# Qervas/cn_chess_ai

Hardware: AMD Instinct MI355X
Metric: env steps/sec + DQN updates/sec at 8192 parallel games, 1/2/4/8 MI355X (higher is better)
Workload: dtype f32

## Files before the change

cn_chess_ai_amd/csrc/xq_dqn.hip:

```cpp
#include "xq_internal.h"
#include <hip/hip_ext.h>
#include "xq_gemm.hip.h"
#include "xq_screen.hip.h"
#include "xq_gemm_dma.hip.h"
#include "xq_l0grad.hip.h"

#include <algorithm>
#include <cfloat>
#include <cmath>
#include <limits>
#include <mutex>
#include <random>
#include <unordered_map>

struct TdStep; struct ScreenPlan;
namespace xq {
struct TailArgs; struct ClipRecord; struct TdStatsRecord; struct ShadowJob;
struct Screen {
    int mode = XQ_QMAX_FULL;
    int refine_stage = -1;
    DevBuf<uint16_t> wb;
    DevBuf<uint16_t> ab;
    DevBuf<float> p1, p2;
    DevBuf<float> R, na;
// ... 89 lines not shown
    xq::DevBuf<float> qsa, yv, lossv;
    xq::DevBuf<uint32_t> gboards;
    int last_n = 0;
    xq::DevBuf<float> grads_td;  size_t n_grads_td = 0;
    size_t g_w0 = 0, g_wh[XQ_MAX_LAYERS] = {0}, g_wout = 0, g_bh[XQ_MAX_LAYERS] = {0}, g_bout = 0;
    xq::DevBuf<float> grads_full;
    int opt_kind = XQ_OPT_SGD;
    double opt_b1 = 0.9, opt_b2 = 0.999, opt_eps = 1e-8;
    uint64_t opt_t = 0;
    xq::DevBuf<float> adam_m, adam_v;
    double clip_max_norm = 0.0;
    xq::DevBuf<double> clip_partials;
    xq::DevBuf<xq::ClipRecord> clip_rec;
    double target_tau = 0.0;
    bool tgt_rest_synced = false;
    int loss_kind = XQ_LOSS_SQUARED;
    double loss_kappa = 1.0;
    float loss_kappa32 = 1.0f;
    xq::DevBuf<xq::TdStatsRecord> td_stats_rec;
    xq::DevBuf<float> slabs;
    xq::DevBuf<float> slabs_l0;
    xq::DevBuf<uint16_t> l0_planes;
    xq::DevBuf<uint16_t> l0_sel;
    bool l0_split_done = false;
    bool l0_sel_done = false;
    bool l0_mfma = true;
    xq_comm* comm = nullptr;
    bool fused_apply = false;
    struct PendingSlab { const float* src = nullptr; int nslabs = 0; long long stride = 0; };
    PendingSlab pend_w0, pend_hidden[XQ_MAX_LAYERS], pend_wout, pend_bout, pend_bh;
    xq::DevBuf<float> bias_work;
    xq::DevBuf<float> xdense, qfull, tfull;
    xq::DevBuf<uint32_t> hb;
    xq::DevBuf<int32_t> ha;  xq::DevBuf<float> hr;  xq::DevBuf<uint8_t> hd;
    xq::StagedBatch staged;
    int bootstrap = XQ_BOOTSTRAP_ALL;
    xq::DevBuf<float> z96, z96_slabs;
    xq::DevBuf<int> legal_nmoves;
    xq::DevBuf<uint8_t> hside;
    int legal_rows = 0;
    int zero_sum = 0;
    int view = XQ_VIEW_ABSOLUTE;
    xq::Profiler prof;
    xq::TailArgs* tail = nullptr;
    bool tail_open = false;
    bool td_tail = true;
// ... 496 lines not shown
    }
    if (kept) { K.valid = true; K.boards = boards_dev; K.n = n; }
    *q90_dev = q;
    *q_stride = 96;
    return XQ_OK;
}

static int check_reference_topology(const xq_dqn* d) {
    for (int l = d->nl - 2; l >= 0; --l) {
        const int inputSize = d->L[l + 1], outputSize = d->L[l];
        if (d->L[l + 2] < inputSize || outputSize < d->L[l + 1] ||
            d->wo[l + 1] + (size_t)(inputSize - 1) * outputSize + (size_t)(d->L[l + 1] - 1) >= d->nw)
            return fail(XQ_ERR_UNDEFINED_UPSTREAM,
                        "bug-compatible backprop reads out of bounds upstream for this topology (layer %d)", l);
    }
    return XQ_OK;
}

static bool l0_mfma_shape(const xq_dqn* d, int n) { return d->l0_mfma && (d->L[1] % 64) == 0 && n >= 256; }
static int l0_chunk_of(int n) { return n >= 16384 ? 2048 : 1024; }
static int ensure_l0_mfma(xq_dqn* d, int n) {
    const int H = d->L[1], chunk = l0_chunk_of(n), kpad = (n + chunk - 1) / chunk * chunk;
    XQ_TRY(reserve_zeroed(d->l0_planes, l0m_plane_elems(H, kpad), d->cur));
    return reserve_zeroed(d->l0_sel, l0sel_elems(kpad), d->cur);
}

static bool grad_bf16_ok(const xq_dqn* d, int M, int N, int K);
static int hidden_deltas(xq_dqn* d, int n, const float* dnext, int ld_next, int k_nz, int mode, int l_start = -1, int l_stop = 0) {
    const float* up = dnext;
    int ld_up = ld_next, nz = k_nz;
    if (l_start < 0) l_start = d->nl - 2;
    for (int l = l_start; l >= l_stop; --l) {
        GemmArgs g; memset(&g, 0, sizeof g);
        g.M = n; g.N = d->L[l + 1];
        const int kfull = (mode == XQ_BACKPROP_REFERENCE) ? d->L[l + 1] : d->L[l + 2];
        g.K = std::min(kfull, nz);
        if (d->bf16_bwd() && up == d->deltas[l + 1] && (n % kBgBM) == 0 && (g.N % kBgBN) == 0 && (g.K % kBgBK) == 0) {
            Bf16GemmArgs b; memset(&b, 0, sizeof b);
            b.M = n; b.N = g.N; b.K = g.K; b.k_chunk = b.K;
            b.A = d->deltas_bf[l + 1]; b.lda = ld_up;
            b.B = d->wl_bf(XQ_NET_ONLINE, l + 1); b.ldb = (mode == XQ_BACKPROP_REFERENCE) ? d->L[l] : d->L[l + 1];
            b.C = d->deltas[l]; b.ldc = d->L[l + 1];
            b.Cb = d->deltas_bf[l]; b.ldcb = d->L[l + 1];
            b.Hb = d->acts_bf[l]; b.ldh = d->L[l + 1];
            XQ_TRY((launch_bf16_gemm<L_KCONTIG, L_MCONTIG, BG_DELTA>(d, b, 1, "gemm_hidden_delta")));
            up = d->deltas[l]; ld_up = d->L[l + 1]; nz = d->L[l + 1];
// ... 127 lines not shown
    s.lds = (size_t)s.nsets * 14 * s.HS * sizeof(float) + (size_t)chunk * sizeof(uint16_t);
    return s;
}

static int l0_gradient(xq_dqn* d, int n, float* dst, xq_dqn::PendingSlab* defer) {
    const int H = d->L[1];
    const int chunk = l0_chunk_of(n);
    const int nchunks = (n + chunk - 1) / chunk;
    const long long len = (long long)kStateSize * H;
    float* out = dst;
    if (nchunks > 1) {
        XQ_TRY(d->slabs_l0.reserve((size_t)nchunks * (size_t)len));
        out = d->slabs_l0;
    }
    if (l0_mfma_shape(d, n)) {
        const int kpad = nchunks * chunk;
        XQ_TRY(ensure_l0_mfma(d, n));
        const size_t need_sel = l0sel_elems(kpad);
        const long long plane_stride = (long long)H * kpad;
        {
            LaunchNow now(d);
            if (!d->l0_sel_done) {
                ProfScope ps(d, "l0_sel_words", 0.0, (double)n * 48 + 2.0 * need_sel);
                hipLaunchKernelGGL(l0_sel_kernel, dim3(kpad / 64), dim3(256), 0, d->cur, d->gboards, n, kpad, d->l0_sel);
            }
            if (!d->l0_split_done) {
                ProfScope ps(d, "l0_delta_split", 8.0 * n * H, (double)n * H * 4 + 6.0 * H * kpad);
                hipLaunchKernelGGL(delta_split_kernel, dim3(kpad / 64, H / 64), dim3(256), 0, d->cur, d->deltas[0], n, H, d->l0_planes, plane_stride, kpad);
            }
            d->l0_sel_done = d->l0_split_done = false;
        }
        XQ_HIP(hipGetLastError());
        const size_t shmem = l0m_lds_bytes();
        const double fl = 2.0 * 80 * 16 * (double)H * kpad * 3, by = 6.0 * H * kpad + 2.0 * need_sel + 4.0 * nchunks * len;
        if (d->tail_open) {
            TailArgs& T = *d->tail;
            T.l0_n = n; T.l0_H = H; T.l0_chunk = chunk; T.l0_nch = nchunks; T.l0_partial = out;
            T.l0_sel = d->l0_sel; T.l0_planes = d->l0_planes; T.l0_plane_stride = plane_stride; T.l0_kpad = kpad; T.l0_ncb = H / kL0mCols;
            T.n_l0 = 4 * (H / kL0mCols) * nchunks;
            d->tail_flops += fl; d->tail_bytes += by;
            d->tail_lds = std::max(d->tail_lds, shmem);
        } else {
            ProfScope ps(d, "l0_grad_segsum", fl, by);
            XQ_TRY(ensure_max_dynamic_lds(l0_grad_mfma_kernel<0>, 64 * 1024));
            hipLaunchKernelGGL(l0_grad_mfma_kernel<0>, dim3(H / kL0mCols, 4, nchunks), dim3(256), shmem, d->cur, d->l0_sel, d->l0_planes, plane_stride,
                               kpad, H, chunk, out);
            XQ_HIP(hipGetLastError());
        }
    } else {
        ProfScope ps(d, "l0_grad_segsum", 2.0 * n * 32 * H, (double)n * (32.0 * H * 4 + 48) + 4.0 * nchunks * len);
        const L0SegShape shape = l0_seg_shape(H, chunk);
        const int HS = shape.HS, nsets = shape.nsets;
        const size_t shmem = shape.lds;
        if (d->tail_open) {
            TailArgs& T = *d->tail;
            T.l0_boards = d->gboards; T.l0_delta = d->deltas[0]; T.l0_n = n; T.l0_H = H; T.l0_HS = HS; T.l0_chunk = chunk; T.l0_nsets = nsets;
            T.l0_nch = nchunks; T.l0_partial = out; T.n_l0 = kSquares * nchunks * (H / HS);
            d->tail_flops += 2.0 * n * 32 * H; d->tail_bytes += (double)n * (32.0 * H * 4 + 48) + 4.0 * nchunks * len;
            d->tail_lds = std::max(d->tail_lds, shmem);
        } else {
        if (shmem > 48 * 1024) XQ_TRY(ensure_max_dynamic_lds(l0_grad_kernel, 64 * 1024));
        hipLaunchKernelGGL(l0_grad_kernel, dim3(kSquares, nchunks, H / HS), dim3(256), shmem, d->cur, d->gboards, d->deltas[0], n, H, HS,
// ... 561 lines not shown
static int side_gradients(xq_dqn* d, const GradPlan& P, int n, float* const* outs, float* G) {
    const int nl = d->nl;
    XQ_TRY(out_gradient(d, P, n, outs[nl - 2], G));
    bool waited = false;
    for (int l = nl - 2; l >= 1; --l) {
        if (l < nl - 2 && !waited) { XQ_HIP(hipStreamWaitEvent(d->cur, d->ev_delta, 0)); waited = true; }
        XQ_TRY(hidden_weight_gradient(d, P, l, n, outs, G));
    }
    if (!waited) XQ_HIP(hipStreamWaitEvent(d->cur, d->ev_delta, 0));
    return hidden_bias_gradients(d, P, n, G);
}

struct TailGrid {
    xq_dqn* d;
    explicit TailGrid(xq_dqn* d_) : d(d_) {
        if (!d->tail) d->tail = new TailArgs();
        memset(d->tail, 0, sizeof(TailArgs));
        d->tail_open = true; d->tail_lds = 0; d->tail_flops = d->tail_bytes = 0;
    }
    ~TailGrid() { d->tail_open = false; }
    int launch(bool last, const char* name) {
        d->tail_open = false;
        const TailArgs& T = *d->tail;
        const long long total = (long long)T.n_l0 + T.n_grad + T.n_delta + T.n_out + T.n_colsum + T.n_sel;
        if (total <= 0) return XQ_OK;
        ProfScope ps(d, name, d->tail_flops, d->tail_bytes, true);
        const auto kern = last ? (T.l0_planes != nullptr ? td_tail_kernel<TAIL_L0 | TAIL_GRAD | TAIL_OUT | TAIL_COLSUM, true>
                                                         : td_tail_kernel<TAIL_L0 | TAIL_GRAD | TAIL_OUT | TAIL_COLSUM>)
                               : (T.n_sel ? td_tail_kernel<TAIL_GRAD | TAIL_DELTA | TAIL_OUT | TAIL_SEL> : td_tail_kernel<TAIL_GRAD | TAIL_DELTA | TAIL_OUT>);
        if (d->tail_lds > 48 * 1024) XQ_TRY(ensure_max_dynamic_lds(kern, 64 * 1024));
        hipExtLaunchKernelGGL(kern, dim3((unsigned)total), dim3(256), d->tail_lds, d->cur, ps.start(), ps.stop(), 0, T);
        XQ_HIP(hipGetLastError());
        return XQ_OK;
    }
};
static bool tail_eligible(xq_dqn* d, int n) {
    if (!d->td_tail || d->bf16()) return false;
    for (int l = 0; l + 2 < d->nl; ++l)
        if (!d->small_tiles && (long long)((n + 127) / 128) * ((d->L[l + 1] + 127) / 128) >= 512) return false;
    return true;
}
static int reduce_pending(xq_dqn* d) {
    SegTable t; memset(&t, 0, sizeof t);
    float* G = d->grads_td;
    int k = 0;
    for_td_segments(d, [&](float*, uint16_t*, size_t goff, long long len, xq_dqn::PendingSlab& p) {
        if (p.nslabs > 0) { t.dst[k] = G + goff; t.src[k] = p.src; t.len[k] = len; t.nslabs[k] = p.nslabs; t.stride[k] = p.stride; ++k; }
        p = xq_dqn::PendingSlab();
    });
    if (k == 0) return XQ_OK;
    t.nseg = k; t.reduce_only = 1;
    return sgd_apply(d, t, 0.0);
}
static int tail_launches(xq_dqn* d, int n, float* const* outs, float* G, int mode) {
    const int nl = d->nl;
    GradPlan P;
    XQ_TRY(plan_gradients(d, n, true, &P));
    const bool defer_grad = nl == 3;
    int waiting = -1;
    for (int l = nl - 3; l >= 0; --l) {
        TailGrid grid(d);
        XQ_TRY(hidden_deltas(d, n, d->deltas[l + 1], d->L[l + 2], d->L[l + 2], mode, l, l));
        if (defer_grad) { if (waiting >= 0) XQ_TRY(hidden_weight_gradient(d, P, waiting, n, outs, G)); waiting = l + 1; }
        else XQ_TRY(hidden_weight_gradient(d, P, l + 1, n, outs, G));
        if (l == nl - 3) XQ_TRY(out_gradient(d, P, n, outs[nl - 2], G));
        if (l == 0 && l0_mfma_shape(d, n)) {
            XQ_TRY(ensure_l0_mfma(d, n));
            TailArgs& T = *d->tail;
            const int chunk0 = l0_chunk_of(n), kpad = (n + chunk0 - 1) / chunk0 * chunk0;
            T.sel_boards = d->gboards; T.sel_n = n; T.sel_kpad = kpad; T.sel_out = d->l0_sel; T.n_sel = kpad / 64;
            d->tail_bytes += (double)n * 48 + 2.0 * l0sel_elems(kpad);
            d->tail_lds = std::max(d->tail_lds, (size_t)64 * 13 * sizeof(uint32_t));
            d->l0_sel_done = true;
        }
        XQ_TRY(grid.launch(false, "td_tail_deltas"));
    }
    TailGrid grid(d);
    XQ_TRY(l0_gradient(d, n, G + d->g_w0, &d->pend_w0));
    if (waiting >= 0) XQ_TRY(hidden_weight_gradient(d, P, waiting, n, outs, G));
    if (nl < 3) XQ_TRY(out_gradient(d, P, n, outs[nl - 2], G));
    XQ_TRY(hidden_bias_gradients(d, P, n, G));
    return grid.launch(true, "td_tail_l0");
}
static int tail_gradients(xq_dqn* d, int n, float* const* outs, float* G, int mode) {
    int rc = tail_launches(d, n, outs, G, mode);
    if (d->late_gate) {
        if (hipEventRecord(d->ev_qmax, d->stream) != hipSuccess && rc == XQ_OK) rc = fail(XQ_ERR_RUNTIME, "hipEventRecord failed");
    }
    if (rc == XQ_OK && !d->fused()) {
        rc = reduce_pending(d);
        if (rc == XQ_OK && d->comm) {
            ProfScope ps(d, "rccl_allreduce_grads", 0, 4.0 * d->n_grads_td);
            rc = comm_allreduce_on(d->comm, G, d->n_grads_td, d->stream);
// ... 1096 lines not shown
```

cn_chess_ai_amd/csrc/xq_l0grad.hip.h:

```cpp
#pragma once

#include "xq_gemm.hip.h"

namespace xq {

constexpr int kL0mRS = 5;
constexpr int kL0mRC = 2;
constexpr int kL0mRowsB = 4 * kL0mRS * 16;
constexpr int kL0mSqB = 24;
constexpr int kL0mCols = 16 * kL0mRC;
constexpr int kL0mStageK = 64;
constexpr int kL0mAPieces = 2 * 3 * kL0mRC;
constexpr int kL0mSPieces = 2 * 3;
constexpr int kL0mStageB = (kL0mAPieces + kL0mSPieces) * 1024;
constexpr int kL0mStages = 3;
constexpr int kL0mSelSquares = 96;

__host__ __device__ constexpr size_t l0m_plane_elems(int H, int kpad) { return (size_t)3 * H * kpad + 8 * 32 + 64; }
__host__ __device__ constexpr size_t l0m_lds_bytes() { return (size_t)kL0mStages * kL0mStageB; }
__host__ __device__ constexpr size_t l0sel_elems(int kpad) { return (size_t)kL0mSelSquares * kpad * 2 + 1024; }

__device__ __forceinline__ void l0_sel_block(const uint32_t* __restrict__ gboards, int n, int kpad, uint16_t* __restrict__ sel, int blk,
                                             uint32_t* __restrict__ bw ) {
    const int tid = (int)threadIdx.x, b0 = blk * 64;
    for (int i = tid; i < 64 * kBoardWords; i += 256) {
        const int s = i / kBoardWords, w = i - s * kBoardWords;
        bw[s * 13 + w] = b0 + s < n ? gboards[(long long)(b0 + s) * kBoardWords + w] : 0u;
    }
    __syncthreads();
    const int octs = kpad >> 3;
    for (int p = tid; p < kL0mSelSquares * 16; p += 256) {
        const int sq = p >> 4, oct = (p >> 1) & 7, enc = p & 1;
        const int wd = sq >> 3, sh = 4 * (sq & 7);
        uint32_t o[4];
#pragma unroll
        for (int i2 = 0; i2 < 4; ++i2) {
            uint32_t v = 0;
#pragma unroll
            for (int e = 0; e < 2; ++e) {
                const uint32_t c = (bw[(oct * 8 + 2 * i2 + e) * 13 + wd] >> sh) & 15u;
                const uint32_t idx = enc ? (c >= 8u ? c - 7u : 0u) : (c <= 7u ? c : 0u);
                v |= idx << (8 + 16 * e);
            }
            o[i2] = v;
        }
        *reinterpret_cast<uint4*>(sel + (((long long)sq * octs + (b0 >> 3) + oct) * 2 + enc) * 8) = make_uint4(o[0], o[1], o[2], o[3]);
    }
}
__global__ __launch_bounds__(256) void l0_sel_kernel(const uint32_t* __restrict__ gboards, int n, int kpad, uint16_t* __restrict__ sel) {
    __shared__ uint32_t bw[64 * 13];
    l0_sel_block(gboards, n, kpad, sel, (int)blockIdx.x, bw);
}

__device__ __forceinline__ void delta_split_block(const float* __restrict__ d0, int n, int H, uint16_t* __restrict__ planes,
                                                   long long plane_stride, int kpad, int tile_k, int tile_c, float* __restrict__ tile ) {
    const int tid = (int)threadIdx.x;
    const int k0 = tile_k * 64, c0 = tile_c * 64;
    {
        const int r = tid >> 4, c4 = (tid & 15) * 4;
#pragma unroll
        for (int i = 0; i < 4; ++i) {
            const int k = k0 + r + 16 * i;
            float4 x = make_float4(0.f, 0.f, 0.f, 0.f);
            if (k < n) x = *reinterpret_cast<const float4*>(d0 + (long long)k * H + c0 + c4);
            float* p = tile + (r + 16 * i) * 65 + c4;
            p[0] = x.x; p[1] = x.y; p[2] = x.z; p[3] = x.w;
        }
    }
    __syncthreads();
    const int col = tid >> 2, kq = (tid & 3) * 16;
    uint32_t w[3][8];
#pragma unroll
    for (int j = 0; j < 16; j += 2) {
        uint32_t pk[3] = {0u, 0u, 0u};
// ... 2 lines not shown
            const float v = tile[(kq + j + e) * 65 + col];
            const uint16_t hi = bf16_bits(0.5f * v);
            const float r1 = 0.5f * v - bf16_to_float(hi);
            const uint16_t mid = bf16_bits(r1);
            const float r2 = r1 - bf16_to_float(mid);
            const uint16_t lo = bf16_bits(r2);
            pk[0] |= (uint32_t)hi << (16 * e); pk[1] |= (uint32_t)mid << (16 * e); pk[2] |= (uint32_t)lo << (16 * e);
        }
        w[0][j >> 1] = pk[0]; w[1][j >> 1] = pk[1]; w[2][j >> 1] = pk[2];
    }
#pragma unroll
    for (int t = 0; t < 3; ++t) {
        uint4* o = reinterpret_cast<uint4*>(planes + t * plane_stride + (long long)(c0 + col) * kpad + k0 + kq);
        o[0] = make_uint4(w[t][0], w[t][1], w[t][2], w[t][3]);
        o[1] = make_uint4(w[t][4], w[t][5], w[t][6], w[t][7]);
    }
}
__global__ __launch_bounds__(256) void delta_split_kernel(const float* __restrict__ d0, int n, int H, uint16_t* __restrict__ planes,
                                                           long long plane_stride, int kpad) {
    __shared__ float tile[64 * 65];
    delta_split_block(d0, n, H, planes, plane_stride, kpad, (int)blockIdx.x, (int)blockIdx.y, tile);
}

template <int DBG = 0>
__device__ __forceinline__ void l0_grad_mfma_block(const uint16_t* __restrict__ sel, const uint16_t* __restrict__ planes,
                                                    long long plane_stride, int kpad, int H, int chunk, float* __restrict__ partial,
                                                    int sqg, int cb, int ch, unsigned char* __restrict__ smem) {
    const int tid = (int)threadIdx.x, lane = tid & 63, wid = __builtin_amdgcn_readfirstlane(tid >> 6);
    const int m = lane & 15, g = lane >> 4;
    const int c0 = ch * chunk, octs = kpad >> 3;
    const unsigned lds0 = (unsigned)(size_t)((__attribute__((address_space(3))) unsigned char*)smem);
    unsigned voff[5];
    int piece[5];
    {
        const int col = lane >> 2, kq = (lane & 3) ^ ((col >> 1) & 3);
#pragma unroll
        for (int i = 0; i < 3; ++i) {
            const int p = wid + 4 * i, kk = p / 6, r = p - 6 * kk, t = r >> 1, c16 = r & 1;
            piece[i] = p;
            voff[i] = (unsigned)((t * plane_stride + (long long)(cb * kL0mCols + c16 * 16 + col) * kpad + c0 + kk * 32 + kq * 8) * 2);
        }
#pragma unroll
        for (int i = 3; i < 5; ++i) {
            const int sp = i == 3 ? wid : 4 + (wid & 1), kk = sp / 3, q = sp - 3 * kk;
            piece[i] = kL0mAPieces + sp;
            const int sq = (sqg * kL0mRowsB) / 14 + q * 8 + (lane >> 3), gg = (lane >> 1) & 3, enc = lane & 1;
            voff[i] = (unsigned)((((long long)sq * octs + (c0 >> 3) + kk * 4 + gg) * 2 + enc) * 16);
        }
    }
    const unsigned char* pA = reinterpret_cast<const unsigned char*>(planes);
    const unsigned char* pS = reinterpret_cast<const unsigned char*>(sel);
    auto issue1 = [&](int st, unsigned buf_off, int i) {
        unsigned keep;
        const unsigned char* base = i < 3 ? pA + (long long)st * (kL0mStageK * 2) : pS + (long long)st * (kL0mStageK / 8 * 32);
        const unsigned l = lds0 + buf_off + (unsigned)piece[i] * 1024u;
        asm volatile("s_mov_b32 %0, m0\n\ts_mov_b32 m0, %3\n\ts_nop 0\n\tglobal_load_lds_dwordx4 %1, %2\n\ts_mov_b32 m0, %0"
                     : "=&s"(keep) : "v"(voff[i]), "s"(base), "s"(l) : "memory");
    };
    auto issue = [&](int st, unsigned buf_off) {
#pragma unroll
        for (int i = 0; i < 5; ++i) issue1(st, buf_off, i);
    };
    issue(0, 0u);
    f32x4 acc[kL0mRC][kL0mRS];
#pragma unroll
    for (int c = 0; c < kL0mRC; ++c)
#pragma unroll
        for (int j = 0; j < kL0mRS; ++j) acc[c][j] = f32x4{0.f, 0.f, 0.f, 0.f};
    uint32_t tlo[kL0mRS], thi[kL0mRS];
    unsigned soff[kL0mRS];
    const unsigned aoff = (unsigned)(m * 64 + ((g ^ ((m >> 1) & 3)) << 4));
    const int sq0 = (sqg * kL0mRowsB) / 14;
#pragma unroll
    for (int j = 0; j < kL0mRS; ++j) {
        const int r = sqg * kL0mRowsB + (wid * kL0mRS + j) * 16 + m;
        const int sq = r / 14, pl = r - sq * 14;
        const int enc = pl >= 7 ? 1 : 0;
        const int idx = r >= kStateSize ? 8 : (enc ? pl - 6 : pl + 1);
        tlo[j] = idx < 4 ? 0x40u << (8 * idx) : 0u;
        thi[j] = (idx >= 4 && idx < 8) ? 0x40u << (8 * (idx - 4)) : 0u;
        const int sl = min(sq - sq0, kL0mSqB - 1);
        soff[j] = (unsigned)((kL0mAPieces + (sl >> 3)) * 1024 + (sl & 7) * 128 + g * 32 + enc * 16);
    }
    struct Frags { bf16x8 a[kL0mRC][3]; uint4 sw[kL0mRS]; };
    constexpr int kReads = 6 + kL0mRS;
    auto read_frag = [&](Frags& f, unsigned boff, int kk, int i) {
        const unsigned char* sp = smem + boff;
        constexpr int kind[kReads] = {0, 1, 1, 0, 1, 1, 0, 1, 1, 0, 0};
        constexpr int arg[kReads] = {0, 0, 1, 1, 2, 3, 2, 4, 5, 3, 4};
        if (kind[i] == 0) f.sw[arg[i]] = *reinterpret_cast<const uint4*>(sp + kk * 3 * 1024 + soff[arg[i]]);
        else f.a[arg[i] & 1][arg[i] >> 1] = *reinterpret_cast<const bf16x8*>(sp + (kk * 6 + arg[i]) * 1024 + aoff);
    };
    auto read_frags = [&](Frags& f, unsigned boff, int kk) {
#pragma unroll
        for (int i = 0; i < kReads; ++i) read_frag(f, boff, kk, i);
    };
    auto onehot2 = [&](int j, uint32_t x, uint32_t y, uint32_t& ox, uint32_t& oy) {
        if (DBG == 3 || DBG == 6) { ox = x; oy = y; }
        else { ox = __builtin_amdgcn_perm(thi[j], tlo[j], x); oy = __builtin_amdgcn_perm(thi[j], tlo[j], y); }
    };
    auto kstep = [&](const Frags& f, const Frags& nxt, uint4& o, auto&& side) {
#pragma unroll
        for (int j = 0; j < kL0mRS; ++j) {
            const bf16x8 b = __builtin_bit_cast(bf16x8, o);
            const uint4 nx = j + 1 < kL0mRS ? f.sw[j + 1] : nxt.sw[0];
            const int jn = j + 1 < kL0mRS ? j + 1 : 0;
            uint4 on;
            if (DBG == 2) {
                asm volatile("" : "+v"(acc[0][j]), "+v"(acc[1][j]) : "v"(f.a[0][0]), "v"(f.a[1][0]), "v"(f.a[0][1]), "v"(f.a[1][1]), "v"(f.a[0][2]), "v"(f.a[1][2]), "v"(b));
                onehot2(jn, nx.x, nx.y, on.x, on.y); onehot2(jn, nx.z, nx.w, on.z, on.w);
                side(3 * j); side(3 * j + 1); side(3 * j + 2);
            } else {
                asm volatile("v_mfma_f32_16x16x32_bf16 %0, %2, %4, %0\n\tv_mfma_f32_16x16x32_bf16 %1, %3, %4, %1"
// ... 8 lines not shown
                __builtin_amdgcn_sched_barrier(0);
                asm volatile("v_mfma_f32_16x16x32_bf16 %0, %2, %4, %0\n\tv_mfma_f32_16x16x32_bf16 %1, %3, %4, %1"
                             : "+v"(acc[0][j]), "+v"(acc[1][j]) : "v"(f.a[0][2]), "v"(f.a[1][2]), "v"(b));
                side(3 * j + 2);
                __builtin_amdgcn_sched_barrier(0);
            }
            o = on;
        }
    };
    const int nst = DBG == 1 ? 0 : chunk / kL0mStageK;
    issue(1, (unsigned)kL0mStageB);
    asm volatile("s_waitcnt vmcnt(5)" ::: "memory");
    __builtin_amdgcn_s_barrier();
    asm volatile("" ::: "memory");
    Frags f0, f1;
    read_frags(f0, 0u, 0);
    if (DBG == 6) read_frags(f1, 0u, 1);
    uint4 o;
    onehot2(0, f0.sw[0].x, f0.sw[0].y, o.x, o.y);
    onehot2(0, f0.sw[0].z, f0.sw[0].w, o.z, o.w);
    asm volatile("s_nop 1" : "+v"(o.x), "+v"(o.y), "+v"(o.z), "+v"(o.w));
    unsigned b_cur = 0u, b_nxt = (unsigned)kL0mStageB, b_far = 2u * kL0mStageB;
    for (int st = 0; st < nst; ++st) {
        kstep(f0, f1, o, [&](int p) {
            if (DBG == 6) return;
            if (p < kReads) read_frag(f1, b_cur, 1, p);
            else if (p < kReads + 4 && DBG != 4) issue1(st + 2, b_far, p - kReads);
        });
        if (DBG != 4 && DBG != 6) asm volatile("s_waitcnt vmcnt(4)" ::: "memory");
        asm volatile("s_waitcnt lgkmcnt(0)" ::: "memory");
        __builtin_amdgcn_s_barrier();
        asm volatile("" ::: "memory");
        kstep(f1, f0, o, [&](int p) {
            if (DBG == 6) return;
            if (p < kReads) read_frag(f0, b_nxt, 0, p);
            else if (p == kReads && DBG != 4) issue1(st + 2, b_far, 4);
        });
        const unsigned t = b_cur; b_cur = b_nxt; b_nxt = b_far; b_far = t;
    }
    asm volatile("s_waitcnt vmcnt(0)\n\ts_nop 7\n\ts_nop 7" ::: "memory");
    {
        float* out = partial + ((long long)ch * kStateSize) * H;
#pragma unroll
        for (int j = 0; j < kL0mRS; ++j) {
            const int r = sqg * kL0mRowsB + (wid * kL0mRS + j) * 16 + m;
            if (r >= kStateSize) continue;
#pragma unroll
            for (int c = 0; c < kL0mRC; ++c) {
                const f32x4 v = acc[c][j];
                *reinterpret_cast<float4*>(out + (long long)r * H + cb * kL0mCols + 16 * c + 4 * g) = make_float4(v[0], v[1], v[2], v[3]);
            }
        }
    }
}

template <int DBG = 0>
__global__ __launch_bounds__(256) void l0_grad_mfma_kernel(const uint16_t* __restrict__ sel, const uint16_t* __restrict__ planes,
                                                            long long plane_stride, int kpad, int H, int chunk, float* __restrict__ partial) {
    extern __shared__ __attribute__((aligned(1024))) unsigned char l0m_smem[];
    l0_grad_mfma_block<DBG>(sel, planes, plane_stride, kpad, H, chunk, partial, (int)blockIdx.y, (int)blockIdx.x, (int)blockIdx.z, l0m_smem);
}

}
```

cn_chess_ai_amd/csrc/xq_tail.hip.h:

```cpp
#pragma once

namespace xq {

__device__ __forceinline__ void out_grad_block(const int32_t* __restrict__ act, const float* __restrict__ dsc,
                                               const float* __restrict__ a_last, int n, int H, int chunk,
                                               float* __restrict__ partial, int g , int chunk_id, float* __restrict__ smem) {
    float* acc = smem;
    uint16_t* list = reinterpret_cast<uint16_t*>(smem + 16 * H);
    __shared__ int total;
    __shared__ float bsum[4][4];
    const int c0 = chunk_id * chunk, c1 = min(n, c0 + chunk);
    const int tid = (int)threadIdx.x, lane = tid & 63, wid = tid >> 6;
    constexpr int kMaxIters = 8;
    __shared__ int wc[kMaxIters][4];
    int clsv[kMaxIters];
#pragma unroll
    for (int it = 0; it < kMaxIters; ++it) {
        const int b = c0 + it * 256 + tid;
        const int a = act[min(b, c1 - 1)];
        clsv[it] = (b < c1 && a >= 4 * g && a < 4 * g + 4) ? a - 4 * g : -1;
    }
    for (int i = tid; i < 16 * H; i += 256) acc[i] = 0.f;
#pragma unroll
    for (int it = 0; it < kMaxIters; ++it) {
// ... 123 lines not shown
    colsum_partial_block(J, (int)blockIdx.x, (int)blockIdx.y, (int)blockIdx.z);
}
__global__ __launch_bounds__(256) void colsum_final_kernel(ColsumJobs J) {
    __shared__ float red[4][64];
    const int job = (int)blockIdx.y;
    const int C = J.C[job];
    const int tx = (int)(threadIdx.x & 63), ty = (int)(threadIdx.x >> 6);
    const int c = (int)blockIdx.x * 64 + tx;
    if ((int)blockIdx.x * 64 >= C) return;
    float s0 = 0.f;
    if (c < C) {
        const float* p = J.work + J.poff[job] + c;
        const int R4 = J.R & ~3;
        for (int z = ty; z < R4; z += 4) s0 += p[(long long)z * J.wld];
        if (ty == 0) for (int z = R4; z < J.R; ++z) s0 += p[(long long)z * J.wld];
    }
    red[ty][tx] = s0;
    __syncthreads();
    if (ty == 0 && c < C) J.dst[job][c] = (red[0][tx] + red[1][tx]) + (red[2][tx] + red[3][tx]);
}

enum { TAIL_DELTA = 1, TAIL_GRAD = 2, TAIL_OUT = 4, TAIL_COLSUM = 8, TAIL_L0 = 16, TAIL_SEL = 32 };
struct TailArgs {
    int n_l0, n_grad, n_delta, n_out, n_colsum, n_sel;
    GemmArgs grad;  int grad_gx, grad_gy;
    GemmArgs delta; int delta_gx;
    const int32_t* og_act; const float* og_dsc; const float* og_alast; int og_n, og_H, og_chunk; float* og_partial;
    const uint32_t* l0_boards; const float* l0_delta; int l0_n, l0_H, l0_HS, l0_chunk, l0_nsets, l0_nch; float* l0_partial;
    const uint16_t* l0_planes; long long l0_plane_stride; int l0_kpad, l0_ncb;
    const uint16_t* l0_sel;
    const uint32_t* sel_boards; int sel_n, sel_kpad; uint16_t* sel_out;
    ColsumJobs cj; int cj_gx, cj_gy;
};
template <unsigned KINDS, bool L0MFMA = false>
__global__ __launch_bounds__(256) void td_tail_kernel(const TailArgs a) {
    extern __shared__ __attribute__((aligned(16))) float tail_smem[];
    int b = (int)blockIdx.x;
    if (KINDS & TAIL_L0) {
        if (b < a.n_l0) {
            if (L0MFMA) {
                int rest = b / a.l0_ncb, cb = b % a.l0_ncb, sqg = rest & 3, ch = rest >> 2;
                if ((a.l0_nch & 7) == 0) { ch = b % a.l0_nch; rest = b / a.l0_nch; cb = rest % a.l0_ncb; sqg = rest / a.l0_ncb; }
                l0_grad_mfma_block<0>(a.l0_sel, a.l0_planes, a.l0_plane_stride, a.l0_kpad, a.l0_H, a.l0_chunk, a.l0_partial, sqg, cb, ch,
                                       reinterpret_cast<unsigned char*>(tail_smem));
                return;
            }
            const int per = kSquares * a.l0_nch;
            l0_grad_block(a.l0_boards, a.l0_delta, a.l0_n, a.l0_H, a.l0_HS, a.l0_chunk, a.l0_nsets, a.l0_partial, b % per, a.l0_nch, b / per, tail_smem);
            return;
        }
        b -= a.n_l0;
    }
    if (KINDS & TAIL_GRAD) {
        if (b < a.n_grad) {
            const int per = a.grad_gx * a.grad_gy, nz = a.n_grad / per, z = b % nz, r = b / nz;
            gemm_f32_block<L_MCONTIG, L_MCONTIG, EPI_STORE, 1, 1>(a.grad, r % a.grad_gx, r / a.grad_gx, z, tail_smem, tail_smem + g_tile_floats(64));
            return;
        }
        b -= a.n_grad;
    }
    if (KINDS & TAIL_DELTA) {
        if (b < a.n_delta) {
            gemm_f32_block<L_KCONTIG, L_MCONTIG, EPI_DELTA, 1, 1>(a.delta, b % a.delta_gx, b / a.delta_gx, 0, tail_smem, tail_smem + g_tile_floats(64));
            return;
        }
        b -= a.n_delta;
    }
    if (KINDS & TAIL_OUT) {
        if (b < a.n_out) {
            out_grad_block(a.og_act, a.og_dsc, a.og_alast, a.og_n, a.og_H, a.og_chunk, a.og_partial, b % 24, b / 24, tail_smem);
            return;
        }
        b -= a.n_out;
    }
    if (KINDS & TAIL_COLSUM) {
        if (b < a.n_colsum) {
            const int per = a.cj_gx * a.cj_gy, r = b % per;
            colsum_partial_block(a.cj, r % a.cj_gx, r / a.cj_gx, b / per);
            return;
        }
        b -= a.n_colsum;
    }
    if (KINDS & TAIL_SEL) {
        if (b < a.n_sel) l0_sel_block(a.sel_boards, a.sel_n, a.sel_kpad, a.sel_out, b, reinterpret_cast<uint32_t*>(tail_smem));
    }
}

}
```

Measured before the change: 49.43 million.

## Restrict layer-0 MFMA gradient to reachable piece-square rows, handle cold rows sparsely

Builds a host table of piece/square input rows that are reachable from the start position under movement rules. The fused-tail layer-0 gradient MFMA kernel then runs over 3 packed groups of hot rows instead of 4 groups covering all 1260 rows. Samples that touch unreachable rows are listed per block, and a small sparse kernel accumulates those rows, or zeroes them when none occur. This cuts MFMA work and adds bookkeeping in the selection kernel plus a new cold-path kernel and pipeline-slot changes.

Measured after the change: 49.98 million, median of 6. 1.01x the previous value.

```diff
diff --git a/cn_chess_ai_amd/csrc/xq_dqn.hip b/cn_chess_ai_amd/csrc/xq_dqn.hip
--- a/cn_chess_ai_amd/csrc/xq_dqn.hip
+++ b/cn_chess_ai_amd/csrc/xq_dqn.hip
@@ -135,6 +135,10 @@
     xq::DevBuf<float> slabs_l0;
     xq::DevBuf<uint16_t> l0_planes;
     xq::DevBuf<uint16_t> l0_sel;
+    xq::DevBuf<uint16_t> l0_hot;
+    xq::DevBuf<uint16_t> l0_cold_list;
+    xq::DevBuf<int> l0_cold_cnt;
+    const xq::L0HotTable* hot() const { return reinterpret_cast<const xq::L0HotTable*>(l0_hot.p); }
     bool l0_split_done = false;
     bool l0_sel_done = false;
     bool l0_mfma = true;
@@ -677,6 +681,14 @@
 static int ensure_l0_mfma(xq_dqn* d, int n) {
     const int H = d->L[1], chunk = l0_chunk_of(n), kpad = (n + chunk - 1) / chunk * chunk;
     XQ_TRY(reserve_zeroed(d->l0_planes, l0m_plane_elems(H, kpad), d->cur));
+    if (!d->l0_hot.p) {
+        const L0HotTable& t = l0_hot_table();
+        if (!t.ok) return fail(XQ_ERR_RUNTIME, "hot-row table: the reachable rows do not fit %d groups of %d", kL0HotGroups, kL0HotGroupRows);
+        XQ_TRY(d->l0_hot.reserve(sizeof(L0HotTable) / sizeof(uint16_t)));
+        XQ_HIP(hipMemcpyAsync(d->l0_hot.p, &t, sizeof t, hipMemcpyHostToDevice, d->cur));
+    }
+    XQ_TRY(d->l0_cold_list.reserve(l0cold_elems(kpad)));
+    XQ_TRY(d->l0_cold_cnt.reserve((size_t)kpad / 64));
     return reserve_zeroed(d->l0_sel, l0sel_elems(kpad), d->cur);
 }
 
@@ -850,7 +862,8 @@
             LaunchNow now(d);
             if (!d->l0_sel_done) {
                 ProfScope ps(d, "l0_sel_words", 0.0, (double)n * 48 + 2.0 * need_sel);
-                hipLaunchKernelGGL(l0_sel_kernel, dim3(kpad / 64), dim3(256), 0, d->cur, d->gboards, n, kpad, d->l0_sel);
+                hipLaunchKernelGGL(l0_sel_kernel, dim3(kpad / 64), dim3(256), 0, d->cur, d->gboards, n, kpad, d->l0_sel, d->hot(), d->l0_cold_list.p,
+                                   d->l0_cold_cnt.p);
             }
             if (!d->l0_split_done) {
                 ProfScope ps(d, "l0_delta_split", 8.0 * n * H, (double)n * H * 4 + 6.0 * H * kpad);
@@ -859,13 +872,17 @@
             d->l0_sel_done = d->l0_split_done = false;
         }
         XQ_HIP(hipGetLastError());
-        const size_t shmem = l0m_lds_bytes();
-        const double fl = 2.0 * 80 * 16 * (double)H * kpad * 3, by = 6.0 * H * kpad + 2.0 * need_sel + 4.0 * nchunks * len;
+        const bool hot = d->tail_open;
+        const size_t shmem = hot ? l0m_lds_bytes<true>() : l0m_lds_bytes<false>();
+        const double fl = 2.0 * (hot ? kL0HotGroups * kL0HotGroupRows : 80 * 16) * (double)H * kpad * 3,
+                     by = 6.0 * H * kpad + 2.0 * need_sel + 4.0 * nchunks * len;
         if (d->tail_open) {
             TailArgs& T = *d->tail;
             T.l0_n = n; T.l0_H = H; T.l0_chunk = chunk; T.l0_nch = nchunks; T.l0_partial = out;
             T.l0_sel = d->l0_sel; T.l0_planes = d->l0_planes; T.l0_plane_stride = plane_stride; T.l0_kpad = kpad; T.l0_ncb = H / kL0mCols;
-            T.n_l0 = 4 * (H / kL0mCols) * nchunks;
+            T.n_l0 = kL0HotGroups * (H / kL0mCols) * nchunks;
+            T.l0_hot = d->hot(); T.l0_cold_list = d->l0_cold_list; T.l0_cold_cnt = d->l0_cold_cnt; T.l0_delta = d->deltas[0];
+            T.n_l0cold = kL0ColdParts * nchunks;
             d->tail_flops += fl; d->tail_bytes += by;
             d->tail_lds = std::max(d->tail_lds, shmem);
         } else {
@@ -1473,7 +1490,7 @@
     int launch(bool last, const char* name) {
         d->tail_open = false;
         const TailArgs& T = *d->tail;
-        const long long total = (long long)T.n_l0 + T.n_grad + T.n_delta + T.n_out + T.n_colsum + T.n_sel;
+        const long long total = (long long)T.n_l0 + T.n_grad + T.n_delta + T.n_out + T.n_colsum + T.n_sel + T.n_l0cold;
         if (total <= 0) return XQ_OK;
         ProfScope ps(d, name, d->tail_flops, d->tail_bytes, true);
         const auto kern = last ? (T.l0_planes != nullptr ? td_tail_kernel<TAIL_L0 | TAIL_GRAD | TAIL_OUT | TAIL_COLSUM, true>
@@ -1520,6 +1537,7 @@
             TailArgs& T = *d->tail;
             const int chunk0 = l0_chunk_of(n), kpad = (n + chunk0 - 1) / chunk0 * chunk0;
             T.sel_boards = d->gboards; T.sel_n = n; T.sel_kpad = kpad; T.sel_out = d->l0_sel; T.n_sel = kpad / 64;
+            T.l0_hot = d->hot(); T.sel_cold_list = d->l0_cold_list; T.sel_cold_cnt = d->l0_cold_cnt;
             d->tail_bytes += (double)n * 48 + 2.0 * l0sel_elems(kpad);
             d->tail_lds = std::max(d->tail_lds, (size_t)64 * 13 * sizeof(uint32_t));
             d->l0_sel_done = true;
diff --git a/cn_chess_ai_amd/csrc/xq_l0grad.hip.h b/cn_chess_ai_amd/csrc/xq_l0grad.hip.h
--- a/cn_chess_ai_amd/csrc/xq_l0grad.hip.h
+++ b/cn_chess_ai_amd/csrc/xq_l0grad.hip.h
@@ -1,37 +1,52 @@
 #pragma once
 
 #include "xq_gemm.hip.h"
+#include "xq_l0hot.h"
 
 namespace xq {
 
-constexpr int kL0mRS = 5;
+template <bool HOT> struct L0mShape {
+    static constexpr int kRS = HOT ? 4 : 5;
+    static constexpr int kRowsB = 4 * kRS * 16;
+    static constexpr int kGroups = HOT ? kL0HotGroups : 4;
+    static constexpr int kSqB = HOT ? kL0HotSqB : 24;
+    static constexpr int kSQ = kSqB / 8;
+    static constexpr int kSPieces = 2 * kSQ;
+    static constexpr int kStageB = (2 * 3 * 2 + kSPieces) * 1024;
+};
+static_assert(L0mShape<true>::kRowsB == kL0HotGroupRows, "the table packs what a block computes");
 constexpr int kL0mRC = 2;
-constexpr int kL0mRowsB = 4 * kL0mRS * 16;
-constexpr int kL0mSqB = 24;
 constexpr int kL0mCols = 16 * kL0mRC;
 constexpr int kL0mStageK = 64;
 constexpr int kL0mAPieces = 2 * 3 * kL0mRC;
-constexpr int kL0mSPieces = 2 * 3;
-constexpr int kL0mStageB = (kL0mAPieces + kL0mSPieces) * 1024;
 constexpr int kL0mStages = 3;
 constexpr int kL0mSelSquares = 96;
 
 __host__ __device__ constexpr size_t l0m_plane_elems(int H, int kpad) { return (size_t)3 * H * kpad + 8 * 32 + 64; }
-__host__ __device__ constexpr size_t l0m_lds_bytes() { return (size_t)kL0mStages * kL0mStageB; }
+template <bool HOT = false> __host__ __device__ constexpr size_t l0m_lds_bytes() { return (size_t)kL0mStages * L0mShape<HOT>::kStageB; }
 __host__ __device__ constexpr size_t l0sel_elems(int kpad) { return (size_t)kL0mSelSquares * kpad * 2 + 1024; }
 
+constexpr int kL0ColdCap = 64 * kSquares;
+constexpr int kL0ColdParts = 8;
+__host__ __device__ constexpr size_t l0cold_elems(int kpad) { return (size_t)(kpad / 64) * kL0ColdCap; }
+
 __device__ __forceinline__ void l0_sel_block(const uint32_t* __restrict__ gboards, int n, int kpad, uint16_t* __restrict__ sel, int blk,
-                                             uint32_t* __restrict__ bw ) {
+                                             uint32_t* __restrict__ bw , const L0HotTable* __restrict__ hot,
+                                             uint16_t* __restrict__ cold_list, int* __restrict__ cold_cnt) {
     const int tid = (int)threadIdx.x, b0 = blk * 64;
+    __shared__ uint16_t hm[kL0mSelSquares];
+    if (tid < kL0mSelSquares) hm[tid] = hot ? hot->hot_mask[tid] : (uint16_t)0x3FFF;
     for (int i = tid; i < 64 * kBoardWords; i += 256) {
         const int s = i / kBoardWords, w = i - s * kBoardWords;
         bw[s * 13 + w] = b0 + s < n ? gboards[(long long)(b0 + s) * kBoardWords + w] : 0u;
     }
     __syncthreads();
     const int octs = kpad >> 3;
+    uint32_t any_cold = 0;
     for (int p = tid; p < kL0mSelSquares * 16; p += 256) {
         const int sq = p >> 4, oct = (p >> 1) & 7, enc = p & 1;
         const int wd = sq >> 3, sh = 4 * (sq & 7);
+        const uint32_t coldp = ~((uint32_t)hm[sq] >> (7 * enc)) << 1;
         uint32_t o[4];
 #pragma unroll
         for (int i2 = 0; i2 < 4; ++i2) {
@@ -41,15 +56,89 @@
                 const uint32_t c = (bw[(oct * 8 + 2 * i2 + e) * 13 + wd] >> sh) & 15u;
                 const uint32_t idx = enc ? (c >= 8u ? c - 7u : 0u) : (c <= 7u ? c : 0u);
                 v |= idx << (8 + 16 * e);
+                any_cold |= idx ? (coldp >> idx) & 1u : 0u;
             }
             o[i2] = v;
         }
         *reinterpret_cast<uint4*>(sel + (((long long)sq * octs + (b0 >> 3) + oct) * 2 + enc) * 8) = make_uint4(o[0], o[1], o[2], o[3]);
     }
-}
-__global__ __launch_bounds__(256) void l0_sel_kernel(const uint32_t* __restrict__ gboards, int n, int kpad, uint16_t* __restrict__ sel) {
+    if (!hot) return;
+    if (!__syncthreads_or((int)any_cold)) {
+        if (tid == 0) cold_cnt[blk] = 0;
+        return;
+    }
+    __shared__ int cc[256];
+    const int s = tid >> 2, sqa = (tid & 3) * 23, sqb = min(kSquares, sqa + 23);
+    auto cold_at = [&](int sq) -> int {
+        const uint32_t c = (bw[s * 13 + (sq >> 3)] >> (4 * (sq & 7))) & 15u;
+        if (c == 0u || c == 15u) return -1;
+        const uint32_t cold_planes = ~(uint32_t)hm[sq] & 0x3FFFu;
+        if (!((cold_planes >> (c - 1u)) & 1u)) return -1;
+        return (int)hot->cold_base[sq] + __popc(cold_planes & ((1u << (c - 1u)) - 1u));
+    };
+    int mine = 0;
+    for (int sq = sqa; sq < sqb; ++sq) mine += cold_at(sq) >= 0;
+    cc[tid] = mine;
+    __syncthreads();
+    int off = 0;
+    for (int i = 0; i < tid; ++i) off += cc[i];
+    uint16_t* lst = cold_list + (long long)blk * kL0ColdCap;
+    for (int sq = sqa; sq < sqb; ++sq) {
+        const int ci = cold_at(sq);
+        if (ci >= 0) lst[off++] = (uint16_t)((s << 10) | ci);
+    }
+    if (tid == 255) cold_cnt[blk] = off;
+}
+__global__ __launch_bounds__(256) void l0_sel_kernel(const uint32_t* __restrict__ gboards, int n, int kpad, uint16_t* __restrict__ sel,
+                                                      const L0HotTable* __restrict__ hot, uint16_t* __restrict__ cold_list,
+                                                      int* __restrict__ cold_cnt) {
     __shared__ uint32_t bw[64 * 13];
-    l0_sel_block(gboards, n, kpad, sel, (int)blockIdx.x, bw);
+    l0_sel_block(gboards, n, kpad, sel, (int)blockIdx.x, bw, hot, cold_list, cold_cnt);
+}
+
+__device__ __forceinline__ void l0_cold_block(const L0HotTable* __restrict__ hot, const uint16_t* __restrict__ cold_list,
+                                              const int* __restrict__ cold_cnt, const float* __restrict__ d0, int H, int chunk,
+                                              float* __restrict__ partial, int ch, int part, int nparts) {
+    const int tid = (int)threadIdx.x, lane = tid & 63, wid = tid >> 6;
+    const int nb = chunk / 64, b0 = ch * nb;
+    int total = 0;
+    for (int i = 0; i < nb; ++i) total += cold_cnt[b0 + i];
+    const int ncold = hot->n_cold, per = (ncold + nparts - 1) / nparts, lo = part * per, hi = min(ncold, lo + per);
+    float* out = partial + (long long)ch * kStateSize * H;
+    if (total == 0) {
+        const int q4 = H >> 2;
+        for (int i = tid; i < (hi - lo) * q4; i += 256) {
+            const int r = hot->cold_row[lo + i / q4];
+            *reinterpret_cast<float4*>(out + (long long)r * H + (i % q4) * 4) = make_float4(0.f, 0.f, 0.f, 0.f);
+        }
+        return;
+    }
+    for (int ci = lo + wid; ci < hi; ci += 4) {
+        const int r = hot->cold_row[ci];
+        for (int cbase = 0; cbase < H; cbase += 256) {
+            const int col = cbase + lane * 4;
+            const bool active = col < H;
+            float4 acc = make_float4(0.f, 0.f, 0.f, 0.f);
+            for (int i = 0; i < nb; ++i) {
+                const int cnt = cold_cnt[b0 + i];
+                const uint16_t* lst = cold_list + (long long)(b0 + i) * kL0ColdCap;
+                for (int e0 = 0; e0 < cnt; e0 += 64) {
+                    const int e = e0 + lane < cnt ? (int)lst[e0 + lane] : 0xFFFF;
+                    unsigned long long mask = __ballot((e & 1023) == ci);
+                    while (mask) {
+                        const int l = __builtin_ctzll(mask);
+                        mask &= mask - 1ull;
+                        const int smp = (b0 + i) * 64 + (__shfl(e, l) >> 10);
+                        if (active) {
+                            const float4 x = *reinterpret_cast<const float4*>(d0 + (long long)smp * H + col);
+                            acc.x += x.x; acc.y += x.y; acc.z += x.z; acc.w += x.w;
+                        }
+                    }
+                }
+            }
+            if (active) *reinterpret_cast<float4*>(out + (long long)r * H + col) = acc;
+        }
+    }
 }
 
 __device__ __forceinline__ void delta_split_block(const float* __restrict__ d0, int n, int H, uint16_t* __restrict__ planes,
@@ -98,10 +187,13 @@
     delta_split_block(d0, n, H, planes, plane_stride, kpad, (int)blockIdx.x, (int)blockIdx.y, tile);
 }
 
-template <int DBG = 0>
+template <int DBG = 0, bool HOT = false>
 __device__ __forceinline__ void l0_grad_mfma_block(const uint16_t* __restrict__ sel, const uint16_t* __restrict__ planes,
                                                     long long plane_stride, int kpad, int H, int chunk, float* __restrict__ partial,
-                                                    int sqg, int cb, int ch, unsigned char* __restrict__ smem) {
+                                                    int sqg, int cb, int ch, unsigned char* __restrict__ smem,
+                                                    const L0HotTable* __restrict__ hot = nullptr) {
+    using Sh = L0mShape<HOT>;
+    constexpr int kL0mRS = Sh::kRS, kL0mRowsB = Sh::kRowsB, kL0mSqB = Sh::kSqB, kL0mSQ = Sh::kSQ, kL0mStageB = Sh::kStageB;
     const int tid = (int)threadIdx.x, lane = tid & 63, wid = __builtin_amdgcn_readfirstlane(tid >> 6);
     const int m = lane & 15, g = lane >> 4;
     const int c0 = ch * chunk, octs = kpad >> 3;
@@ -118,9 +210,10 @@
         }
 #pragma unroll
         for (int i = 3; i < 5; ++i) {
-            const int sp = i == 3 ? wid : 4 + (wid & 1), kk = sp / 3, q = sp - 3 * kk;
+            const int sp = i == 3 ? wid : 4 + (HOT ? wid : (wid & 1)), kk = sp / kL0mSQ, q = sp - kL0mSQ * kk;
             piece[i] = kL0mAPieces + sp;
-            const int sq = (sqg * kL0mRowsB) / 14 + q * 8 + (lane >> 3), gg = (lane >> 1) & 3, enc = lane & 1;
+            const int sqb = HOT ? (int)hot->sq0[sqg] : (sqg * kL0mRowsB) / 14;
+            const int sq = min(sqb + q * 8 + (lane >> 3), kL0mSelSquares - 1), gg = (lane >> 1) & 3, enc = lane & 1;
             voff[i] = (unsigned)((((long long)sq * octs + (c0 >> 3) + kk * 4 + gg) * 2 + enc) * 16);
         }
     }
@@ -146,11 +239,12 @@
     uint32_t tlo[kL0mRS], thi[kL0mRS];
     unsigned soff[kL0mRS];
     const unsigned aoff = (unsigned)(m * 64 + ((g ^ ((m >> 1) & 3)) << 4));
-    const int sq0 = (sqg * kL0mRowsB) / 14;
+    const int sq0 = HOT ? (int)hot->sq0[sqg] : (sqg * kL0mRowsB) / 14;
 #pragma unroll
     for (int j = 0; j < kL0mRS; ++j) {
-        const int r = sqg * kL0mRowsB + (wid * kL0mRS + j) * 16 + m;
-        const int sq = r / 14, pl = r - sq * 14;
+        const int pr = sqg * kL0mRowsB + (wid * kL0mRS + j) * 16 + m;
+        const int r = HOT ? (int)hot->row[pr] : pr;
+        const int sq = r >= kStateSize ? sq0 : r / 14, pl = r >= kStateSize ? 0 : r - sq * 14;
         const int enc = pl >= 7 ? 1 : 0;
         const int idx = r >= kStateSize ? 8 : (enc ? pl - 6 : pl + 1);
         tlo[j] = idx < 4 ? 0x40u << (8 * idx) : 0u;
@@ -160,11 +254,12 @@
     }
     struct Frags { bf16x8 a[kL0mRC][3]; uint4 sw[kL0mRS]; };
     constexpr int kReads = 6 + kL0mRS;
+    static_assert(kL0mRS == 4 || kL0mRS == 5, "the read order below lists tiles 0..4");
     auto read_frag = [&](Frags& f, unsigned boff, int kk, int i) {
         const unsigned char* sp = smem + boff;
-        constexpr int kind[kReads] = {0, 1, 1, 0, 1, 1, 0, 1, 1, 0, 0};
-        constexpr int arg[kReads] = {0, 0, 1, 1, 2, 3, 2, 4, 5, 3, 4};
-        if (kind[i] == 0) f.sw[arg[i]] = *reinterpret_cast<const uint4*>(sp + kk * 3 * 1024 + soff[arg[i]]);
+        constexpr int kind[11] = {0, 1, 1, 0, 1, 1, 0, 1, 1, 0, 0};
+        constexpr int arg[11] = {0, 0, 1, 1, 2, 3, 2, 4, 5, 3, 4};
+        if (kind[i] == 0) f.sw[arg[i]] = *reinterpret_cast<const uint4*>(sp + kk * kL0mSQ * 1024 + soff[arg[i]]);
         else f.a[arg[i] & 1][arg[i] >> 1] = *reinterpret_cast<const bf16x8*>(sp + (kk * 6 + arg[i]) * 1024 + aoff);
     };
     auto read_frags = [&](Frags& f, unsigned boff, int kk) {
@@ -219,19 +314,26 @@
     asm volatile("s_nop 1" : "+v"(o.x), "+v"(o.y), "+v"(o.z), "+v"(o.w));
     unsigned b_cur = 0u, b_nxt = (unsigned)kL0mStageB, b_far = 2u * kL0mStageB;
     for (int st = 0; st < nst; ++st) {
+        constexpr int kSlots = 3 * kL0mRS, kDma0 = kSlots - kReads < 5 ? kSlots - kReads : 5;
         kstep(f0, f1, o, [&](int p) {
             if (DBG == 6) return;
             if (p < kReads) read_frag(f1, b_cur, 1, p);
-            else if (p < kReads + 4 && DBG != 4) issue1(st + 2, b_far, p - kReads);
+            else if (p < kReads + kDma0 && DBG != 4) issue1(st + 2, b_far, p - kReads);
         });
-        if (DBG != 4 && DBG != 6) asm volatile("s_waitcnt vmcnt(4)" ::: "memory");
+        if (DBG != 4 && DBG != 6) asm volatile("s_waitcnt vmcnt(%0)" :: "n"(kDma0) : "memory");
         asm volatile("s_waitcnt lgkmcnt(0)" ::: "memory");
         __builtin_amdgcn_s_barrier();
         asm volatile("" ::: "memory");
         kstep(f1, f0, o, [&](int p) {
             if (DBG == 6) return;
-            if (p < kReads) read_frag(f0, b_nxt, 0, p);
-            else if (p == kReads && DBG != 4) issue1(st + 2, b_far, 4);
+            if (p < kReads) { read_frag(f0, b_nxt, 0, p); return; }
+            if (DBG == 4) return;
+            const int i = kDma0 + p - kReads;
+            if (i < 5) issue1(st + 2, b_far, i);
+            if (p == kSlots - 1) {
+#pragma unroll
+                for (int i2 = 0; i2 < 5; ++i2) if (i2 > i) issue1(st + 2, b_far, i2);
+            }
         });
         const unsigned t = b_cur; b_cur = b_nxt; b_nxt = b_far; b_far = t;
     }
@@ -240,7 +342,8 @@
         float* out = partial + ((long long)ch * kStateSize) * H;
 #pragma unroll
         for (int j = 0; j < kL0mRS; ++j) {
-            const int r = sqg * kL0mRowsB + (wid * kL0mRS + j) * 16 + m;
+            const int pr = sqg * kL0mRowsB + (wid * kL0mRS + j) * 16 + m;
+            const int r = HOT ? (int)hot->row[pr] : pr;
             if (r >= kStateSize) continue;
 #pragma unroll
             for (int c = 0; c < kL0mRC; ++c) {
diff --git a/cn_chess_ai_amd/csrc/xq_l0hot.h b/cn_chess_ai_amd/csrc/xq_l0hot.h
--- /dev/null
+++ b/cn_chess_ai_amd/csrc/xq_l0hot.h
@@ -0,0 +1,100 @@
+#pragma once
+
+#include <cstdint>
+#include <cstring>
+
+namespace xq {
+
+constexpr int kL0HotGroups = 3;
+constexpr int kL0HotGroupRows = 256;
+constexpr int kL0HotSqB = 32;
+constexpr uint16_t kL0NoRow = 0xFFFF;
+constexpr uint16_t kL0ColdBit = 0x8000;
+
+struct L0HotTable {
+    uint16_t row[kL0HotGroups * kL0HotGroupRows];
+    uint16_t index[1260];
+    uint16_t cold_row[1260];
+    uint16_t hot_mask[96];
+    uint16_t cold_base[96];
+    uint16_t sq0[kL0HotGroups + 1];
+    uint16_t n_hot, n_cold, ok, pad_;
+};
+
+namespace l0hot_detail {
+inline bool any_palace(int r, int c) { return c >= 3 && c <= 5 && ((r >= 0 && r <= 2) || (r >= 7 && r <= 9)); }
+inline bool rule(int code, int fr, int fc, int tr, int tc) {
+    if ((unsigned)tr >= 10u || (unsigned)tc >= 9u) return false;
+    const int type = code > 7 ? code - 7 : code;
+    const int dr = tr - fr, dc = tc - fc, adr = dr < 0 ? -dr : dr, adc = dc < 0 ? -dc : dc;
+    switch (type) {
+        case 1: return any_palace(fr, fc) && any_palace(tr, tc) && adr + adc == 1;
+        case 2: return any_palace(tr, tc) && adr == 1 && adc == 1;
+        case 3: return adr == 2 && adc == 2 && ((fr < 5 && tr < 5) || (fr >= 5 && tr >= 5));
+        case 4: return (adr == 2 && adc == 1) || (adr == 1 && adc == 2);
+        case 5: case 6: return (fr == tr) != (fc == tc);
+        case 7:
+            if (code <= 7) return fr < 5 ? (dr == 1 && adc == 0) : ((dr == 1 && adc == 0) || (dr == 0 && adc == 1));
+            return fr >= 5 ? (dr == -1 && adc == 0) : ((dr == -1 && adc == 0) || (dr == 0 && adc == 1));
+        default: return false;
+    }
+}
+}
+
+inline void l0_hot_build(L0HotTable* t) {
+    using namespace l0hot_detail;
+    memset(t, 0, sizeof *t);
+    static const uint8_t back[9] = {5, 4, 3, 2, 1, 2, 3, 4, 5};
+    uint8_t start[90] = {0};
+    for (int c = 0; c < 9; ++c) { start[c] = back[c]; start[81 + c] = (uint8_t)(back[c] + 7); }
+    start[19] = start[25] = 6; start[64] = start[70] = 13;
+    for (int c = 0; c < 9; c += 2) { start[27 + c] = 7; start[54 + c] = 14; }
+    bool hot[1260] = {false};
+    for (int s = 0; s < 90; ++s) if (start[s]) hot[s * 14 + start[s] - 1] = true;
+    for (bool grew = true; grew;) {
+        grew = false;
+        for (int code = 1; code <= 14; ++code)
+            for (int s = 0; s < 90; ++s) {
+                if (!hot[s * 14 + code - 1]) continue;
+                for (int d = 0; d < 90; ++d)
+                    if (d != s && !hot[d * 14 + code - 1] && rule(code, s / 9, s % 9, d / 9, d % 9)) hot[d * 14 + code - 1] = grew = true;
+            }
+    }
+    for (int i = 0; i < kL0HotGroups * kL0HotGroupRows; ++i) t->row[i] = kL0NoRow;
+    for (int i = 0; i < 1260; ++i) t->cold_row[i] = kL0NoRow;
+    int g = 0, in_rows = 0, in_sq = 0, n_hot = 0, n_cold = 0;
+    bool fits = true;
+    t->sq0[0] = 0;
+    for (int s = 0; s < 90; ++s) {
+        int h = 0;
+        for (int p = 0; p < 14; ++p) h += hot[s * 14 + p];
+        if (in_rows + h > kL0HotGroupRows || in_sq == kL0HotSqB) {
+            if (++g >= kL0HotGroups) { fits = false; break; }
+            t->sq0[g] = (uint16_t)s; in_rows = in_sq = 0;
+        }
+        t->cold_base[s] = (uint16_t)n_cold;
+        for (int p = 0; p < 14; ++p) {
+            const int r = s * 14 + p;
+            if (hot[r]) {
+                t->hot_mask[s] |= (uint16_t)(1u << p);
+                t->index[r] = (uint16_t)(g * kL0HotGroupRows + in_rows);
+                t->row[g * kL0HotGroupRows + in_rows++] = (uint16_t)r;
+                ++n_hot;
+            } else {
+                t->index[r] = (uint16_t)(kL0ColdBit | n_cold);
+                t->cold_row[n_cold++] = (uint16_t)r;
+            }
+        }
+        ++in_sq;
+    }
+    for (int k = g + 1; k <= kL0HotGroups; ++k) t->sq0[k] = 90;
+    for (int s = 90; s < 96; ++s) t->cold_base[s] = (uint16_t)n_cold;
+    t->n_hot = (uint16_t)n_hot; t->n_cold = (uint16_t)n_cold; t->ok = fits ? 1 : 0;
+}
+
+inline const L0HotTable& l0_hot_table() {
+    static const L0HotTable* t = [] { L0HotTable* p = new L0HotTable; l0_hot_build(p); return p; }();
+    return *t;
+}
+
+}
diff --git a/cn_chess_ai_amd/csrc/xq_tail.hip.h b/cn_chess_ai_amd/csrc/xq_tail.hip.h
--- a/cn_chess_ai_amd/csrc/xq_tail.hip.h
+++ b/cn_chess_ai_amd/csrc/xq_tail.hip.h
@@ -169,14 +169,17 @@
 
 enum { TAIL_DELTA = 1, TAIL_GRAD = 2, TAIL_OUT = 4, TAIL_COLSUM = 8, TAIL_L0 = 16, TAIL_SEL = 32 };
 struct TailArgs {
-    int n_l0, n_grad, n_delta, n_out, n_colsum, n_sel;
+    int n_l0, n_grad, n_delta, n_out, n_colsum, n_sel, n_l0cold;
     GemmArgs grad;  int grad_gx, grad_gy;
     GemmArgs delta; int delta_gx;
     const int32_t* og_act; const float* og_dsc; const float* og_alast; int og_n, og_H, og_chunk; float* og_partial;
     const uint32_t* l0_boards; const float* l0_delta; int l0_n, l0_H, l0_HS, l0_chunk, l0_nsets, l0_nch; float* l0_partial;
     const uint16_t* l0_planes; long long l0_plane_stride; int l0_kpad, l0_ncb;
     const uint16_t* l0_sel;
+    const L0HotTable* l0_hot;
+    const uint16_t* l0_cold_list; const int* l0_cold_cnt;
     const uint32_t* sel_boards; int sel_n, sel_kpad; uint16_t* sel_out;
+    uint16_t* sel_cold_list; int* sel_cold_cnt;
     ColsumJobs cj; int cj_gx, cj_gy;
 };
 template <unsigned KINDS, bool L0MFMA = false>
@@ -186,10 +189,10 @@
     if (KINDS & TAIL_L0) {
         if (b < a.n_l0) {
             if (L0MFMA) {
-                int rest = b / a.l0_ncb, cb = b % a.l0_ncb, sqg = rest & 3, ch = rest >> 2;
+                int rest = b / a.l0_ncb, cb = b % a.l0_ncb, sqg = rest % kL0HotGroups, ch = rest / kL0HotGroups;
                 if ((a.l0_nch & 7) == 0) { ch = b % a.l0_nch; rest = b / a.l0_nch; cb = rest % a.l0_ncb; sqg = rest / a.l0_ncb; }
-                l0_grad_mfma_block<0>(a.l0_sel, a.l0_planes, a.l0_plane_stride, a.l0_kpad, a.l0_H, a.l0_chunk, a.l0_partial, sqg, cb, ch,
-                                       reinterpret_cast<unsigned char*>(tail_smem));
+                l0_grad_mfma_block<0, true>(a.l0_sel, a.l0_planes, a.l0_plane_stride, a.l0_kpad, a.l0_H, a.l0_chunk, a.l0_partial, sqg, cb, ch,
+                                             reinterpret_cast<unsigned char*>(tail_smem), a.l0_hot);
                 return;
             }
             const int per = kSquares * a.l0_nch;
@@ -197,6 +200,14 @@
             return;
         }
         b -= a.n_l0;
+        if (L0MFMA) {
+            if (b < a.n_l0cold) {
+                l0_cold_block(a.l0_hot, a.l0_cold_list, a.l0_cold_cnt, a.l0_delta, a.l0_H, a.l0_chunk, a.l0_partial, b / kL0ColdParts,
+                              b % kL0ColdParts, kL0ColdParts);
+                return;
+            }
+            b -= a.n_l0cold;
+        }
     }
     if (KINDS & TAIL_GRAD) {
         if (b < a.n_grad) {
@@ -229,8 +240,12 @@
         b -= a.n_colsum;
     }
     if (KINDS & TAIL_SEL) {
-        if (b < a.n_sel) l0_sel_block(a.sel_boards, a.sel_n, a.sel_kpad, a.sel_out, b, reinterpret_cast<uint32_t*>(tail_smem));
-    }
-}
-
-}
+        if (b < a.n_sel) {
+            l0_sel_block(a.sel_boards, a.sel_n, a.sel_kpad, a.sel_out, b, reinterpret_cast<uint32_t*>(tail_smem), a.l0_hot, a.sel_cold_list,
+                         a.sel_cold_cnt);
+            return;
+        }
+    }
+}
+
+}
```
